# jzebedee/deltaq

Hardware: AMD Instinct MI355X
Metric: MB of text suffix-sorted per second (bit-exact SA) (higher is better)
Workload: dtype u8 text / u64 keys / int32 SA; 1 GPU; 256 MiB uniform-random bytes per GPU (splitmix64 seed 0x5EED0003+rank), int32 SA; bytes_per_gpu=268435456, residency=text and SA resident in HBM, rounds_after_initial_sort=1

## Files before the change

### deltaq_amd/csrc/dq_flags.h

```cpp
#pragma once

#include <algorithm>
#include <cstdint>
#include <cstdlib>
#include <cstring>
#include <optional>
#include <string>

namespace dq {

struct Flags {
    bool debug = false;
    std::optional<int> trace;
    std::optional<int> hip_device;
    std::optional<int> numa_bind;
    std::optional<std::string> fault;
    std::optional<int> small_n;
    std::optional<int> no_many;
    std::optional<int> mid_many_min;
    std::optional<int> no_large_many;
    std::optional<int> large_many_min;
    std::optional<int> no_diff_many;
    std::optional<int> no_diff_mid_many;
    std::optional<int> diff_mid_many_min;
    std::optional<int> no_diff_large;
    std::optional<int> diff_large_min;
    std::optional<int> diff_large_table;
    std::optional<int> no_index_many;
    std::optional<int> index_many_min;
    std::optional<int> index_many_threads;
    std::optional<int> no_index_large;
    std::optional<int> index_large_min;
    std::optional<int> no_check_many;
    std::optional<int> no_bwt_many;
    std::optional<int> no_mtf_many;
    std::optional<int> no_huff_many;
    std::optional<int> mtf_short_max;
    std::optional<int> unbz2_one_start;
    bool no_list_buffers = false;
    bool text_copy = false;
    bool assume_doubled = false;
    bool no_twins = false;
    bool no_period_hint = false;
    std::optional<int> xcd_group;
    std::optional<int> packed;
    std::optional<int> key_bytes;
    std::optional<int> coded;
    std::optional<int> split;
    bool no_bucket = false;
    std::optional<int> bucket;
    std::optional<int> bucket_keybits;
    std::optional<int> bucket_ext;
    std::optional<int> bucket_tile;
    std::optional<int> bucket_slots;
    std::optional<int> tie_settle;
    bool old_first_pass = false;
    bool no_fused_ties = false;
    std::optional<int> sparse;
    std::optional<int> binned_isa;
    bool no_binned_isa = false;
    std::optional<int> runs;
    bool no_small = false;
    bool no_wide_small = false;
    bool no_first_small = false;
    std::optional<int> mid_groups;
    bool no_l_shift = false;
    bool no_upd_words = false;
    std::optional<int> upd_bin;
    std::optional<int> upd_bin_min;
    std::optional<int> upd_window;
    std::optional<int> chain_steps;
    bool no_chain = false;
    bool force_rshift = false;
    std::optional<int> tail_max;
    std::optional<int> pair_chains;
    std::optional<int> pair_chains_min;
    std::optional<int> pair_maxg;
    std::optional<int> late_runs_min;
    bool no_late_runs = false;
    std::optional<int> run_period;
    bool search_wave = false;
    std::optional<int> search_ptab;
    bool no_wave_windows = false;
    bool no_poll = false;
    bool no_second_stage = false;
    std::optional<int> win_min;
    std::optional<int> win_second;
// ... 45 lines not shown
    f.no_diff_mid_many = num("DQ_NO_DIFF_MID_MANY", 0, 1);
    f.diff_mid_many_min = num("DQ_DIFF_MID_MANY_MIN", 1);
    f.no_diff_large = num("DQ_NO_DIFF_LARGE", 0, 1);
    f.diff_large_min = num("DQ_DIFF_LARGE_MIN", 1);
    f.diff_large_table = num("DQ_DIFF_LARGE_TABLE", 0, 1);
    f.no_index_many = num("DQ_NO_INDEX_MANY", 0, 1);
    f.index_many_min = num("DQ_INDEX_MANY_MIN", 1);
    f.index_many_threads = num("DQ_INDEX_MANY_THREADS");
    f.no_index_large = num("DQ_NO_INDEX_LARGE", 0, 1);
    f.index_large_min = num("DQ_INDEX_LARGE_MIN", 1);
    f.no_check_many = num("DQ_NO_CHECK_MANY", 0, 1);
    f.no_bwt_many = num("DQ_NO_BWT_MANY", 0, 1);
    f.no_mtf_many = num("DQ_NO_MTF_MANY", 0, 1);
    f.no_huff_many = num("DQ_NO_HUFF_MANY", 0, 1);
    f.mtf_short_max = num("DQ_MTF_SHORT_MAX", 0);
    f.unbz2_one_start = num("DQ_UNBZ2_ONE_START", 0, 1);
    f.no_list_buffers = on("DQ_NO_LIST_BUFFERS");
    f.text_copy = on("DQ_TEXT_COPY");
    f.assume_doubled = on("DQ_ASSUME_DOUBLED");
    f.no_twins = on("DQ_NO_TWINS");
    f.no_period_hint = on("DQ_NO_PERIOD_HINT");

    f.xcd_group = num("DQ_XCD_GROUP", 0, 64);
    f.packed = num("DQ_PACKED");
    f.key_bytes = num("DQ_KEY_BYTES", 1, 8);
    f.coded = num("DQ_CODED");
    f.split = num("DQ_SPLIT");
    f.no_bucket = on("DQ_NO_BUCKET");
    f.bucket = num("DQ_BUCKET");
    f.bucket_keybits = num("DQ_BUCKET_KEYBITS");
    f.bucket_ext = num("DQ_BUCKET_EXT");
    f.bucket_tile = num("DQ_BUCKET_TILE", 0, 1);
    f.bucket_slots = num("DQ_BUCKET_SLOTS", 0, 1);
    f.tie_settle = num("DQ_TIE_SETTLE", 0, 1);
    f.old_first_pass = on("DQ_OLD_FIRST_PASS");
    f.no_fused_ties = on("DQ_NO_FUSED_TIES");
    f.sparse = num("DQ_SPARSE");
    f.binned_isa = num("DQ_BINNED_ISA");
    f.no_binned_isa = on("DQ_NO_BINNED_ISA");
    f.runs = num("DQ_RUNS");

    f.no_small = on("DQ_NO_SMALL");
    f.no_wide_small = on("DQ_NO_WIDE_SMALL");
    f.no_first_small = on("DQ_NO_FIRST_SMALL");
    f.mid_groups = num("DQ_MID_GROUPS");
    f.no_l_shift = on("DQ_NO_L_SHIFT");
    f.no_upd_words = on("DQ_NO_UPD_WORDS");
    f.upd_bin = num("DQ_UPD_BIN", 0, 2);
    f.upd_bin_min = num("DQ_UPD_BIN_MIN", 1);
    f.upd_window = num("DQ_UPD_WINDOW");
    f.chain_steps = num("DQ_CHAIN_STEPS");
    f.no_chain = on("DQ_NO_CHAIN");
    f.force_rshift = on("DQ_FORCE_RSHIFT");

    f.tail_max = num("DQ_TAIL_MAX", 0);
    f.pair_chains = num("DQ_PAIR_CHAINS");
    f.pair_chains_min = num("DQ_PAIR_CHAINS_MIN", 1);
    f.pair_maxg = num("DQ_PAIR_MAXG", 2);
    f.late_runs_min = num("DQ_LATE_RUNS_MIN", 1);
    f.no_late_runs = on("DQ_NO_LATE_RUNS");
    f.run_period = num("DQ_RUN_PERIOD", 1);

    f.search_wave = on("DQ_SEARCH_WAVE");
    f.search_ptab = num("DQ_SEARCH_PTAB");
    f.no_wave_windows = on("DQ_NO_WAVE_WINDOWS");
    f.no_poll = on("DQ_NO_POLL");
// ... 79 lines not shown
```

### deltaq_amd/csrc/dq_round0.h

```cpp
#pragma once
#include "dq_sort_passes.h"
#include "dq_alpha_code.h"
#include "dq_ties.h"
#include "dq_bucket_sort.h"
#include "dq_xcd_rank.h"
#include "dq_slot_rank.h"

namespace dq {
namespace {

constexpr int64_t kSgShortList = 1 << 20;
inline int mid_group_cap(int64_t list_len)
{
    if (const std::optional<int> g = flags().mid_groups) {
        return *g >= 1024 ? 1024 : *g >= 512 ? 512 : *g >= 256 ? 256 : 0;
    }
    return list_len >= kSgShortList ? 512 : 1024;
}
inline bool small_round_usable(int64_t n, int64_t mm, bool third_list_buffer)
{
    const Flags &F = flags();
    return !F.no_small && n < (1ll << 32) && (mm * 2 <= n || (third_list_buffer && !F.no_wide_small));
}

// ... 45 lines not shown
    int digit_tables(int kb, bool coded_keys)
    {
        if (coded_keys) {
            const int hblocks = (int)std::min<int64_t>(kHistBlocks, ((n >> 2) + kHistThreads - 1) / kHistThreads + 1);
            DQ_TRY(L.begin(DQ_K_RADIX_HIST, n, n));
            HIP_TRY(hipMemsetAsync(w.hist_partial, 0, (size_t)kMaxPasses * kRadixSize * 8, st));
            hipLaunchKernelGGL(text_coded_hist_kernel, dim3(hblocks), dim3(kHistThreads), 0, st,
                               reinterpret_cast<const uint32_t *>(w.text), n, (const uint16_t *)w.codetab,
                               reinterpret_cast<unsigned long long *>(w.hist_partial));
            hipLaunchKernelGGL(radix_hist_scan_kernel, dim3(kMaxPasses), dim3(kHistScanThreads), 0, st,
                               (const unsigned long long *)w.hist_partial, w.digit_offset);
            HIP_TRY(hipGetLastError());
            return L.end();
        }
        hipLaunchKernelGGL(text_digit_offsets_kernel, dim3(kb), dim3(kBlock), 0, st,
                           (const int64_t *)w.bytehist, (const uint8_t *)w.text, n, kb, w.digit_offset);
        HIP_TRY(hipGetLastError());
        return DQ_OK;
    }

    int prepare()
    {
        int blocks = (int)std::min<int64_t>(1024, ((n >> 4) + kBlock - 1) / kBlock + 1);
        unsigned long long *xcd_hist = n >= kRound0MinN ? reinterpret_cast<unsigned long long *>(w.bytehist + kXcdHistAt) : nullptr;
        if (xcd_hist) blocks = (blocks + kXcds - 1) / kXcds * kXcds;
        HIP_TRY(hipMemsetAsync(w.bytehist, 0, (size_t)(kXcdHistAt + (xcd_hist ? kXcds * kRadixSize : 0)) * 8, L.st));
        LAUNCH(L, DQ_K_TEXT_HIST, n, n,
               hipLaunchKernelGGL(text_hist_kernel, dim3(blocks + 1), dim3(kBlock), 0, L.st,
                                  text_src ? text_src : (const uint8_t *)w.text, n, reinterpret_cast<unsigned long long *>(w.bytehist),
                                  reinterpret_cast<unsigned long long *>(w.bytehist + 256), text_src ? w.text : (uint8_t *)nullptr,
                                  xcd_hist));
        HIP_TRY(hipMemcpyAsync(c.pinned, w.bytehist, (256 + 10) * 8, hipMemcpyDeviceToHost, L.st));
        HIP_TRY(hipEventRecord(c.readback, L.st));
        constexpr int kEarlyPasses = 3;
        DQ_TRY(prepare_status<IdxT>(L, w, n, kEarlyPasses));
        if (n >= kRound0MinN) HIP_TRY(hipMemsetAsync(w.Vb, 0, (size_t)(tie_words() + 1) * 8, L.st));
        HIP_TRY(hipEventSynchronize(c.readback));
        const Flags &F = flags();
        s = TextStats(c.pinned, n);
        ib = s.ib;
        k = choose_key_bytes(s, F);
        DQ_TRY(prepare_status<IdxT>(L, w, n, k.kb, kEarlyPasses));
        bool hist_deferred = false;
        if (coded_keys_tried(s, F, k)) {
            AlphaCode code;
            if (build_alpha_code(s.hist, &code) && (code.avg_len <= kCodedMaxAvgLen || F.coded)) {
                uint16_t *stage = reinterpret_cast<uint16_t *>(c.pinned + 512);
                memcpy(stage, code.tab, sizeof(code.tab));
                HIP_TRY(hipMemcpyAsync(w.codetab, stage, sizeof(code.tab), hipMemcpyHostToDevice, L.st));
                coded = true;
                hist_deferred = split_round0_wanted(n, k, (int)wb, F);
                if (F.trace) fprintf(stderr, "[dq] coded round 0: %d symbols, %.2f bits per byte\n", code.sigma, code.avg_len);
            }
        }
        if (hist_deferred) return DQ_OK;
        if (!coded && plan_bucketed(s, F, k, coded, (int)wb).applies) return DQ_OK;
        return digit_tables(k.kb, coded);
    }

    int passes(int &cur, uint32_t *ebits = nullptr, uint64_t *seam_tab = nullptr)
    {
        const int kb = k.kb;
        if (k.packed) {
            DQ_TRY(rank_pass<IdxT, kTextPacked>(L, w, text64(), (const IdxT *)nullptr, K[1], (IdxT *)nullptr, n, 0, kb, ib));
            cur = 1;
            for (int p = 1; p < kb; ++p) {
                if (p == kb - 1 && ebits)
                    DQ_TRY(rank_pass<IdxT, kKeysLastTies>(L, w, K[cur], (const IdxT *)nullptr, (uint64_t *)nullptr, d_sa, n, p,
                                                          kb, ib, ebits, seam_tab));
                else if (p == kb - 1)
                    DQ_TRY(rank_pass<IdxT, kKeysLast>(L, w, K[cur], (const IdxT *)nullptr, K[cur ^ 1], d_sa, n, p, kb, ib));
                else
                    DQ_TRY(rank_pass<IdxT, kKeys>(L, w, K[cur], (const IdxT *)nullptr, K[cur ^ 1], (IdxT *)nullptr, n, p, kb, ib));
                cur ^= 1;
            }
            return DQ_OK;
        }
        DQ_TRY(with_bool(coded, [&](auto kCoded) -> int {
            return rank_pass<IdxT, kText, decltype(kCoded)::value>(L, w, text64(), (const IdxT *)nullptr, K[1], V[1], n, 0, kb);
        }));
        cur = 1;
        for (int p = 1; p < kb; ++p) {
            DQ_TRY(rank_pass<IdxT, kPairs>(L, w, K[cur], V[cur], K[cur ^ 1], V[cur ^ 1], n, p, kb));
            cur ^= 1;
        }
        return DQ_OK;
    }

    int collect_ties(uint32_t *ebits, const uint64_t *seam_tab, uint64_t *act_rank, bool *overflow, uint64_t *fin_rank,
                     bool seams = true, int64_t h_fin = -1, bool settle = false)
// ... 102 lines not shown
                                  keys, w.Va, cnt));
        o.keys_ready = with_key2;
        o.list_ungrouped = true;
        return DQ_OK;
    }

    int bucketed(bool *done)
    {
        *done = false;
        const Flags &F = flags();
        const BucketPlan b = plan_bucketed(s, F, k, coded, (int)wb);
        if (!b.applies) return DQ_OK;
        const int kb = k.kb, keybits = b.keybits, lowbits = b.lowbits;
        const SlotPlan sp = bucket_slots_fit(s, b, (int)wb);
        const FinishTiles ft = plan_finish_tiles(b, n, F, sp.fits);
        static_assert(sizeof(SlotRankCtl) <= (size_t)kHistBlocks * kMaxPasses * kRadixSize * 4, "the cursors live in the histogram scratch");
        const bool slots = bucket_slots_wanted(sp, ft, F) && (uint64_t)sp.words <= slot_span_words_of(w) &&
                           (size_t)(2 * kSlotBuckets + 5) * 4 <= finish_bounds_entries(n) * 8;
        uint32_t *slot_base = reinterpret_cast<uint32_t *>(w.bkt_bounds), *slot_out = slot_base + kSlotBuckets + 4;
        SlotRankCtl *sctl = reinterpret_cast<SlotRankCtl *>(w.hist_partial);
        const int first = slots ? 0 : 1;
        uint8_t *E[2] = {reinterpret_cast<uint8_t *>(w.Va), reinterpret_cast<uint8_t *>(w.Va) + align_up((size_t)n)};
        uint32_t *ebits = reinterpret_cast<uint32_t *>(w.Vb);
        TieCounters *ctr = reinterpret_cast<TieCounters *>(w.totals + 6);
        BucketFlags *bflags = reinterpret_cast<BucketFlags *>(&ctr->overflow);
        hipLaunchKernelGGL(text_digit_offsets_kernel, dim3(b.bbytes), dim3(kBlock), 0, st,
                           (const int64_t *)w.bytehist, (const uint8_t *)w.text, n, b.bbytes, w.digit_offset,
                           b.xcd_pass ? (const int64_t *)(w.bytehist + kXcdHistAt) : nullptr, b.xcd_pass ? w.xcd_offset : nullptr);
        HIP_TRY(hipGetLastError());
        if (slots) {
            if (F.trace)
                fprintf(stderr, "[dq] second pass into bucket slots: %d x %d slots of %lld words (n=%lld)\n", sp.first, sp.second,
                        (long long)b.X, (long long)n);
            HIP_TRY(hipMemsetAsync(sctl, 0, sizeof(SlotRankCtl), st));
            hipLaunchKernelGGL(slot_plan_kernel, dim3(kRadixSize + 1), dim3(kBlock), 0, st, (const int64_t *)w.bytehist, b.X, slot_base);
            HIP_TRY(hipGetLastError());
        }
        if (c.ncu <= 0) {
            int v = 0;
            c.ncu = hipDeviceGetAttribute(&v, hipDeviceAttributeMultiprocessorCount, c.dev) == hipSuccess && v > 0 ? v : 256;
        }
        if (b.xcd_pass) {
            if (F.trace) fprintf(stderr, "[dq] XCD-local first pass (n=%lld, eighths of %lld)\n", (long long)n, (long long)xcd_eighth(n));
            if (sizeof(XcdRankCtl) > w.ctl_status_stride) return fail(DQ_ERR_HIP, "status buffer too small");
            LAUNCH(L, DQ_K_RADIX_RANK, n, n * (1 + 8),
                   hipLaunchKernelGGL(xcd_text_rank_kernel, dim3((unsigned)std::min<int64_t>(c.ncu, (n + kXcdTileN - 1) / kXcdTileN)),
                                      dim3(kXcdRankThreads), 0, st, reinterpret_cast<const uint32_t *>(w.text), K[first], n,
                                      ib + lowbits, keybits, ib, (const int64_t *)w.xcd_offset,
                                      reinterpret_cast<XcdRankCtl *>(w.ctl_status)));
        } else {
            DQ_TRY(b.ext ? rank_pass_ext<IdxT, kTextPackedExt>(L, w, text64(), (const uint8_t *)nullptr, K[1], E[1], n, 0, ib, ib + lowbits, keybits)
                       : rank_pass<IdxT, kTextPacked>(L, w, text64(), (const IdxT *)nullptr, K[first], (IdxT *)nullptr, n, 0, kb, ib,
                                                      nullptr, nullptr, ib + lowbits, keybits));
        }
        if (slots) {
            const int groups = resident_groups(&c.slot_rank_groups, (const void *)slot_rank_kernel, kSlotRankThreads, c.dev);
            LAUNCH(L, DQ_K_RADIX_RANK, n, n * 16,
                   hipLaunchKernelGGL(slot_rank_kernel, dim3((unsigned)std::min<int64_t>(groups, (n + kSlotTileN - 1) / kSlotTileN)),
                                      dim3(kSlotRankThreads), 0, st, (const uint64_t *)K[0], K[1], n, ib + lowbits + 8, ib + lowbits,
                                      (const int64_t *)w.digit_offset, (const uint32_t *)slot_base, sctl, bflags));
        }
        for (int p = 1; p < b.bbytes && !slots; ++p) {
            DQ_TRY(b.ext ? rank_pass_ext<IdxT, kKeysExt>(L, w, K[p & 1], E[p & 1], K[(p & 1) ^ 1], E[(p & 1) ^ 1], n, p, ib, ib + lowbits + 8 * p, keybits)
                       : rank_pass<IdxT, kKeys>(L, w, K[p & 1], (const IdxT *)nullptr, K[(p & 1) ^ 1], (IdxT *)nullptr, n, p, kb, ib,
                                                nullptr, nullptr, ib + lowbits + 8 * p, keybits));
        }
        uint64_t *Ks = slots ? K[1] : K[b.bbytes & 1], *Kfree = slots ? K[0] : K[(b.bbytes & 1) ^ 1];
        const uint8_t *Es = b.ext ? E[b.bbytes & 1] : nullptr;
        if (F.trace)
            fprintf(stderr, "[dq] bucket finish: %s geometry, %lld tiles of up to %lld words cut every %lld %s (n=%lld)\n", ft.fine ? "fine" : "coarse",
                    (long long)ft.ntiles, (long long)ft.cap, (long long)(ft.by_id ? ft.g : ft.Cf), ft.by_id ? "buckets" : "words", (long long)n);
        if ((size_t)ft.ntiles + 1 > finish_bounds_entries(n)) return fail(DQ_ERR_HIP, "tile bounds buffer too small");
        if (slots) {
            LAUNCH(L, DQ_K_BUCKET_SORT, ft.ntiles, ft.ntiles * 16,
                   hipLaunchKernelGGL(slot_out_kernel, dim3(kRadixSize), dim3(kSlotOutThreads), 0, st, sctl->cursor, (uint32_t)b.X,
                                      (const int64_t *)(w.digit_offset + kRadixSize) , n, slot_out, bflags));
            auto kernel = bucket_sort_kernel<IdxT, false, BktFine, true>;
            const int groups = resident_groups(&c.bkt_slot_groups[sizeof(IdxT) == 8], (const void *)kernel, BktFine::threads, c.dev);
            LAUNCH(L, DQ_K_BUCKET_SORT, n, n * (8 + wb) + n / 8,
                   hipLaunchKernelGGL(kernel, dim3((unsigned)std::min<int64_t>(ft.ntiles, groups)), dim3(BktFine::threads), 0, st,
                                      (const uint64_t *)Ks, ib, lowbits, (const int64_t *)nullptr, ft.ntiles, d_sa, ebits, bflags,
                                      (const uint8_t *)nullptr, (const uint32_t *)slot_base, (const uint32_t *)sctl->cursor, (const uint32_t *)slot_out));
        } else if (ft.by_id) {
            const int64_t nbuckets = (int64_t)1 << (8 * b.bbytes);
            LAUNCH(L, DQ_K_BUCKET_SORT, ft.ntiles, ft.ntiles * 16 * 8,
                   hipLaunchKernelGGL(bucket_bounds_by_id_kernel, dim3((unsigned)((nbuckets + 1 + kBlock - 1) / kBlock)), dim3(kBlock), 0,
                                      st, (const uint64_t *)Ks, n, ib + lowbits, ft.g, b.X, nbuckets, ft.ntiles, w.bkt_bounds, bflags));
        } else {
            LAUNCH(L, DQ_K_BUCKET_SORT, ft.ntiles, ft.ntiles * 16 * 8,
                   hipLaunchKernelGGL(bucket_bounds_kernel, dim3((unsigned)((ft.ntiles + 1 + kBlock - 1) / kBlock)), dim3(kBlock), 0,
                                      st, (const uint64_t *)Ks, n, ib + lowbits, ft.Cf, b.X, ft.ntiles, w.bkt_bounds, bflags));
        }
        auto finish = [&](auto kExt, auto geometry) -> int {
// ... 151 lines not shown
            }
            *done = true;
            return DQ_OK;
        }
    }

    int run()
    {
        const Flags &F = flags();
        int cur = 0;
        DQ_TRY(prepare());
        const int kb = k.kb;
        o.runs = plan_runs(s, F, (int)wb, period_hint);
        V[kb & 1] = d_sa;
        V[(kb & 1) ^ 1] = w.Va;
        o.Vr[0] = w.Va; o.Vr[1] = w.Vb;
        o.rbits = ib;
        o.h = kb;
        bool done = false;
        DQ_TRY(bucketed(&done));
        if (done) return DQ_OK;
        if (fused_ties_wanted(n, k, F)) {
            uint32_t *ebits = reinterpret_cast<uint32_t *>(w.Vb);
            uint64_t *seam_tab = reinterpret_cast<uint64_t *>(reinterpret_cast<char *>(w.Vb) +
                                                              align_up((size_t)(tie_words() + 1) * 8));
            DQ_TRY(passes(cur, ebits, seam_tab));
            bool overflow = false;
            DQ_TRY(collect_ties(ebits, seam_tab, K[cur], &overflow, K[cur ^ 1]));
            o.fin_done = !overflow && o.m <= o.fin_cap;
            if (!overflow) {
                o.Kr[0] = K[cur]; o.Kr[1] = K[cur ^ 1];
                return DQ_OK;
            }
            HIP_TRY(hipMemsetAsync(w.ctl_status + (size_t)(kb - 1) * w.ctl_status_stride, 0, w.ctl_status_stride, st));
            DQ_TRY(rank_pass<IdxT, kKeysLast>(L, w, K[cur ^ 1], (const IdxT *)nullptr, K[cur], d_sa, n, kb - 1, kb, ib));
        } else {
            bool split_done = false;
            const bool split_wanted = split_round0_wanted(n, k, (int)wb, F);
            if (split_wanted && (!o.runs.runs_wanted || F.split)) {
                DQ_TRY(split(&split_done));
            }
            if (split_wanted && !split_done) {
                DQ_TRY(digit_tables(kb, coded));
                DQ_TRY(prepare_status<IdxT>(L, w, n, kb));
            }
            if (split_done) {
                cur = 1;
            } else {
                DQ_TRY(passes(cur));
            }
        }
        const int kshift0 = k.packed ? ib : 0;
        const DenseGuess guess = dense_guess(n, k);
        int64_t tied_pairs = 0;
        if (guess == DenseGuess::kTakeSample) {
            HIP_TRY(hipMemsetAsync(w.totals + 2, 0, 8, st));
            hipLaunchKernelGGL(sample_ties_kernel, dim3(kTieSamples / kBlock), dim3(kBlock), 0, st,
                               (const uint64_t *)K[cur], n, kshift0, kTieSamples, w.totals + 2);
            HIP_TRY(hipGetLastError());
            HIP_TRY(hipMemcpyAsync(c.pinned, w.totals + 2, 8, hipMemcpyDeviceToHost, st));
            HIP_TRY(hipStreamSynchronize(st));
            tied_pairs = c.pinned[0];
        }
        o.dense_built = predict_dense(guess, tied_pairs, F);
        if (o.dense_built && binned_isa_pays(n, F)) {
            o.Kr[0] = K[cur]; o.Kr[1] = K[cur ^ 1];
            return build_isa_binned(K[cur], K[cur ^ 1], kshift0);
// ... 10 lines not shown
```

### deltaq_amd/csrc/dq_round0_plan.h

```cpp
#pragma once
#include <algorithm>
#include <cmath>
#include <cstddef>
#include <cstdint>

#include "dq_flags.h"

namespace dq {

constexpr int kKgramSamples = 1024;
constexpr int kBktCap = 12288;
constexpr int kBktCapFine = 6144;
constexpr int kSplitTop = 512;
constexpr int kSplitSub = 512;
constexpr int kSplitBuckets = kSplitTop * kSplitSub;
constexpr int kFinCap = 2048;
constexpr int64_t kSplitMinN = 5ll << 20;
constexpr int64_t kCodedMinN = 8ll << 20;
constexpr double kCodedMaxAvgLen = 5.8;
constexpr int kTieSamples = 4096;
constexpr int64_t kRound0MinN = 1 << 16;

inline int index_bits(int64_t n) { return n <= 1 ? 1 : 64 - __builtin_clzll((uint64_t)(n - 1)); }

// ... 160 lines not shown
};

inline SlotPlan bucket_slots_fit(const TextStats &s, const BucketPlan &b, int idx_bytes)
{
    SlotPlan p;
    if (!b.applies || b.bbytes != 2 || b.ext) return p;
    p.first = s.sigma;
    p.second = s.sigma + (s.hist[0] == 0 ? 1 : 0);
    p.words = (int64_t)p.first * p.second * b.X;
    p.fits = p.words <= slot_span_words(s.n, idx_bytes) && p.words < ((int64_t)1 << 32);
    return p;
}

inline void slot_bases(const int64_t *hist , int64_t X, uint32_t *base )
{
    int ra[257], rb[257];
    ra[0] = rb[0] = 0;
    for (int d = 0; d < 256; ++d) {
        ra[d + 1] = ra[d] + (hist[d] > 0 ? 1 : 0);
        rb[d + 1] = rb[d] + (hist[d] > 0 || d == 0 ? 1 : 0);
    }
    for (int A = 0; A < 256; ++A)
        for (int B = 0; B < 256; ++B)
            base[A * 256 + B] = (uint32_t)(X * ((int64_t)ra[A] * rb[256] + (hist[A] > 0 ? rb[B] : 0)));
    base[65536] = (uint32_t)(X * ra[256] * rb[256]);
}

inline bool bucket_slots_wanted(const SlotPlan &p, const FinishTiles &t, const Flags &F)
{
    if (F.bucket_slots && *F.bucket_slots == 0) return false;
    return p.fits && t.fine && t.by_id && t.g == 1;
}

inline size_t finish_bounds_entries(int64_t n)
{
    const size_t by_words = (size_t)n / (kBktCapFine / 2) + 4;
    return n < kRound0MinN ? by_words : std::max<size_t>(by_words, 65536 + 4);
}

inline bool fused_ties_wanted(int64_t n, KeyPlan k, const Flags &F)
{
    return k.packed && k.kb >= 2 && n >= kRound0MinN && !F.no_fused_ties && !F.sparse;
}

enum class DenseGuess { kNeither, kGuessDense, kTakeSample };

inline DenseGuess dense_guess(int64_t n, KeyPlan k)
{
    if (n < kRound0MinN || k.packed || k.kb != 8) return DenseGuess::kNeither;
    return n < (8 << 20) ? DenseGuess::kGuessDense : DenseGuess::kTakeSample;
}

inline bool predict_dense(DenseGuess g, int64_t tied_pairs, const Flags &F)
{
    if (F.sparse) return *F.sparse == 0;
    return g == DenseGuess::kGuessDense || (g == DenseGuess::kTakeSample && tied_pairs * 12 > kTieSamples);
}

inline bool binned_isa_pays(int64_t n, const Flags &F)
{
    const bool pays = F.binned_isa ? *F.binned_isa != 0 : n > (32ll << 20);
    return pays && n >= kRound0MinN && 2 * index_bits(n) <= 63 && !F.no_binned_isa;
}

struct RunPlan {
    bool runs_wanted = false;
// ... 18 lines not shown
```

### deltaq_amd/csrc/dq_slot_rank.h

```cpp
#pragma once
#include "dq_bucket_sort.h"
#include "dq_xcd_rank.h"

namespace dq {

constexpr int kSlotBuckets = 1 << 16;

struct SlotRankCtl {
    uint32_t ticket[kXcds];
    uint32_t pad[64 - kXcds];
    uint32_t cursor[kSlotBuckets];
};

static __global__ __launch_bounds__(kBlock) void slot_plan_kernel(const int64_t *__restrict__ bytehist, int64_t X,
                                                           uint32_t *__restrict__ slot_base )
{
    __shared__ int tmp[kWavesPerBlock];
    __shared__ int s_rank, s_present;
    const int d = threadIdx.x, A = blockIdx.x;
    const int pa = bytehist[d] > 0 ? 1 : 0, pb = (pa || d == 0) ? 1 : 0;
    int na, nb;
    const int ra = block_excl_sum(pa, tmp, &na);
    __syncthreads();
    const int rb = block_excl_sum(pb, tmp, &nb);
    if (A == kRadixSize) {
        if (d == 0) slot_base[kSlotBuckets] = (uint32_t)(X * na * nb);
        return;
    }
    if (d == A) { s_rank = ra; s_present = pa; }
    __syncthreads();
    slot_base[A * kRadixSize + d] = (uint32_t)(X * ((int64_t)s_rank * nb + (s_present ? rb : 0)));
}

constexpr int kSlotOutThreads = kRadixSize;
static __global__ __launch_bounds__(kSlotOutThreads) void slot_out_kernel(uint32_t *__restrict__ count , uint32_t X,
                                                                   const int64_t *__restrict__ first_offset , int64_t n,
                                                                   uint32_t *__restrict__ out ,
                                                                   BucketFlags *__restrict__ flags)
{
    static_assert(kSlotOutThreads == kBlock, "block_excl_sum scans kBlock values");
    __shared__ uint32_t tmp[kWavesPerBlock];
    const int A = blockIdx.x, B = threadIdx.x;
    int64_t lo = first_offset[A], hi = A + 1 < kRadixSize ? first_offset[A + 1] : n;
    lo = lo < 0 ? 0 : (lo > n ? n : lo);
    hi = hi < lo ? lo : (hi > n ? n : hi);
    const uint32_t room = (uint32_t)(hi - lo);
    const uint32_t raw = count[A * kRadixSize + B];
    const uint32_t c = min(raw, X);
    uint32_t total;
    const uint32_t excl = block_excl_sum(c, tmp, &total);
    const uint32_t place = min(excl, room);
    const uint32_t kept = min(c, room - place);
    if (kept != raw) {
        atomicOr(&flags->overflow, 2ull);
        count[A * kRadixSize + B] = kept;
    }
    out[A * kRadixSize + B] = (uint32_t)lo + place;
    if (A == kRadixSize - 1 && B == kRadixSize - 1) out[kSlotBuckets] = (uint32_t)n;
}

#ifdef DQ_SLOT_PHASE_TIMING
__device__ long long *g_slot_ts = nullptr;
__device__ unsigned int g_slot_ts_next = 0;
#define DQ_SLOT_PHASE(i) do { if (threadIdx.x == 0 && g_slot_ts) g_slot_ts[(long long)ts_row * 8 + (i)] = clock64(); } while (0)
#else
#define DQ_SLOT_PHASE(i) do { } while (0)
#endif

constexpr int kSlotRankThreads = 1024;
constexpr int kSlotRankItems = 12;
constexpr int kSlotTileN = kSlotRankThreads * kSlotRankItems;

static __global__ __launch_bounds__(kSlotRankThreads, 1) void slot_rank_kernel(
    const uint64_t *__restrict__ kin , uint64_t *__restrict__ wout, int64_t n,
    int shift , int bshift ,
    const int64_t *__restrict__ region , const uint32_t *__restrict__ slot_base ,
    SlotRankCtl *__restrict__ ctl, BucketFlags *__restrict__ flags)
{
    constexpr int kThreads = kSlotRankThreads, kItems = kSlotRankItems, kTileN = kSlotTileN;
    constexpr int kPerXcd = kRadixSize / kXcds;
    __shared__ __attribute__((aligned(16))) uint64_t exch[kTileN];
    __shared__ uint32_t cnt[kRadixSize];
    __shared__ uint32_t tile_base[kRadixSize];
    __shared__ uint32_t gofs[kRadixSize];
    __shared__ uint32_t glim[kRadixSize];
    __shared__ uint32_t wtmp[kRadixSize / kWave];
    __shared__ uint32_t r_lo[kRadixSize], r_hi[kRadixSize], r_tiles[kRadixSize];
    __shared__ uint32_t xs[kXcds][kPerXcd + 1];
    __shared__ uint32_t s_lo, s_cnt;

    const int tid = threadIdx.x;
    const int w = tid >> 6;
    const int lane = lane_id();
    const uint32_t xcd = hw_xcc_id();

    if (tid < kRadixSize) {
        const int64_t lo = region[tid], hi = tid + 1 < kRadixSize ? region[tid + 1] : n;
        r_lo[tid] = (uint32_t)lo;
        r_hi[tid] = (uint32_t)hi;
        r_tiles[tid] = (uint32_t)((hi - lo + kTileN - 1) / kTileN);
        cnt[tid] = 0;
    }
    __syncthreads();
    if (tid < kXcds) {
        uint32_t run = 0;
        for (int j = 0; j < kPerXcd; ++j) { xs[tid][j] = run; run += r_tiles[tid + kXcds * j]; }
        xs[tid][kPerXcd] = run;
    }
    __syncthreads();

    int tried = 0;
    int32_t pend_e = -1;
// ... 121 lines not shown
```

### deltaq_amd/csrc/dq_sort_passes.h

```cpp
#pragma once
#include "dq_runtime.h"
#include "dq_round0_plan.h"
#include "dq_onesweep.h"
#include "dq_radix.h"
#include "dq_sa_kernels.h"
#include "dq_seg_fused.h"
#include "dq_small_groups.h"
#include "dq_runs.h"
#include "dq_isa_pairs.h"
#include "dq_split_round0.h"

namespace dq {
namespace {

constexpr int kSgChain = 8;

inline unsigned grid_for(int64_t items)
{
    return (unsigned)std::min<int64_t>((items + kBlock - 1) / kBlock, 256 * 16);
}

constexpr int64_t kSmallTileMaxM = 1ll << 20;
inline bool small_tiles(int64_t m) { return m <= kSmallTileMaxM; }
inline size_t status_tiles(size_t m)
{
    const size_t small = (m < (size_t)kSmallTileMaxM ? m : (size_t)kSmallTileMaxM) / 2048;
    return std::max(m / 8192, small) + 2;
}

template <typename IdxT>
struct Workspace {
    uint8_t *text;
    uint64_t *K0, *K1;
    IdxT *Va, *Vb, *ISA, *SAbuf;
    uint64_t *X;
    IdxT *Xs;
    int64_t *bkt_bounds;
    int64_t *totals;
    SmallGroupCounters *sg_ctr;
    uint32_t *hist_partial;
    uint16_t *codetab;
    uint32_t *pc_tiles;
    uint32_t *RL;
    uint32_t *run_lead, *run_carry;
    uint8_t *run_link;
    int64_t *digit_offset;
    int64_t *bytehist;
    int64_t *xcd_offset;
    char *ctl_status;
    size_t ctl_status_bytes;
    size_t ctl_status_stride;
    char *seg_status;
    size_t seg_status_bytes;
    uint64_t *sp_top, *sp_sub;
    unsigned long long *sp_cnt_a, *sp_cursor_a, *sp_cursor_b;
    int64_t *sp_off, *sp_out_base, *sp_ovf_src, *sp_ovf_dst;
    uint64_t *sp_low;
    uint8_t *sp_pure;
    uint32_t *sp_tile_first;
    ScanPart *sp_part;
    SplitCtl *sp_ctl;
    size_t slot_span_words;
    size_t bytes;
};

template <typename IdxT>
inline uint64_t slot_span_words_of(const Workspace<IdxT> &w) { return (uint64_t)w.slot_span_words; }

template <typename IdxT>
Workspace<IdxT> carve(char *base, int64_t n, bool with_sa, bool lists)
{
    Workspace<IdxT> w{};
    size_t off = 0;
    auto take = [&](size_t b) { char *p = base ? base + off : nullptr; off += align_up(b); return p; };
    const size_t un = (size_t)n;
    w.text = (uint8_t *)take(un + 64);
    w.K0 = (uint64_t *)take((un + 2) * 8);
    const size_t k1_at = off;
    w.K1 = (uint64_t *)take((un + 2) * 8);
    const bool adjacent = off == k1_at + align_up((un + 2) * 8);
    w.Va = (IdxT *)take((un + 2) * sizeof(IdxT));
    w.slot_span_words = adjacent ? (off - k1_at) / 8 : 0;
    w.Vb = (IdxT *)take((un + 2) * sizeof(IdxT));
    w.ISA = (IdxT *)take(un * sizeof(IdxT));
// ... 31 lines not shown
        w.sp_off = (int64_t *)take((size_t)(kSplitTop + 1) * 8);
        w.sp_out_base = (int64_t *)take((size_t)(kSplitBuckets + 1) * 8);
        w.sp_ovf_src = (int64_t *)take((size_t)kSplitBuckets * 8);
        w.sp_ovf_dst = (int64_t *)take((size_t)kSplitBuckets * 8);
        w.sp_low = (uint64_t *)take((size_t)kSplitBuckets * 8);
        w.sp_pure = (uint8_t *)take((size_t)kSplitBuckets);
        w.sp_tile_first = (uint32_t *)take((size_t)(kSplitTop + 1) * 4);
        w.sp_part = (ScanPart *)take((size_t)kScanBlocks * sizeof(ScanPart));
        w.sp_ctl = (SplitCtl *)take(sizeof(SplitCtl));
    }
    w.bytes = off;
    return w;
}

constexpr uint64_t kWsReserve = 1ull << 30;

template <typename IdxT>
bool with_list_buffers(int64_t n, bool with_sa, uint64_t avail)
{
    return n < (1ll << 32) && carve<IdxT>(nullptr, n, with_sa, true).bytes <= avail;
}

template <typename IdxT, int kMode, bool kSmall = false> struct RankCfg {
    static constexpr bool kExtra = (kMode == kTextPackedExt || kMode == kKeysExt);
    static constexpr bool kWords = (kMode == kTextPacked || kMode == kKeys || kMode == kKeysLast || kMode == kKeysLastTies || kExtra);
    static constexpr int kThreads = kSmall ? 256 : 512;
    static constexpr int kItems = kSmall ? 8 : kExtra ? 20 : kWords ? 24 : (sizeof(IdxT) == 4 ? 20 : 16);
    static constexpr int kMinWaves = 2;
    static constexpr int kRounds = 2;
    static constexpr bool kLdsMatch = kWords;
    static constexpr bool kAtomicBase = (kMode == kTextPacked || kMode == kText || kMode == kTextPackedExt);
};

template <typename IdxT>
int prepare_status(Launcher &L, Workspace<IdxT> &w, int64_t m, int passes, int from = 0)
{
    const size_t word = m < (1ll << 30) ? 4 : 8;
    const size_t stride = align_up(256 + status_tiles((size_t)m) * kRadixSize * word);
    if ((size_t)passes * stride > w.ctl_status_bytes) return fail(DQ_ERR_HIP, "status buffer too small");
    w.ctl_status_stride = stride;
    if (passes > from) HIP_TRY(hipMemsetAsync(w.ctl_status + (size_t)from * stride, 0, (size_t)(passes - from) * stride, L.st));
    return DQ_OK;
}

inline uint32_t spin_bound() { return t_fault.spin ? 0u : kSpinLimit; }

inline int xcd_tile_group() { return flags().xcd_group.value_or(8); }

template <typename IdxT, typename StatusT, int kMode, bool kCoded = false, bool kSmall = false>
int launch_rank_pass(Launcher &L, Workspace<IdxT> &w, const uint64_t *kin, const IdxT *vin,
                     uint64_t *kout, IdxT *vout, int64_t m, int pass, int kb, int ib,
                     uint32_t *ebits = nullptr, uint64_t *seam_tab = nullptr, int shift_override = -1,
                     int keybits = 0)
{
    using Cfg = RankCfg<IdxT, kMode, kSmall>;
    constexpr int kItems = Cfg::kItems;
    constexpr int kThreads = Cfg::kThreads;
    constexpr int kTileN = kThreads * kItems;
    const int64_t ntiles = (m + kTileN - 1) / kTileN;
    const int64_t wb = (int64_t)sizeof(IdxT);
    char *area = w.ctl_status + (size_t)pass * w.ctl_status_stride;
    OnesweepCtl *ctl = reinterpret_cast<OnesweepCtl *>(area);
    StatusT *status = reinterpret_cast<StatusT *>(area + 256);
    if (256 + (size_t)ntiles * kRadixSize * sizeof(StatusT) > w.ctl_status_stride)
        return fail(DQ_ERR_HIP, "status buffer too small");
    const int64_t alg = kMode == kPairs ? 2 * (8 + wb) : kMode == kText ? 1 + 8 + wb
                      : kMode == kTextPacked ? 1 + 8 : kMode == kKeys ? 16 : kMode == kKeysLastTies ? 8 + wb : 16 + wb;
    const int64_t alg_extra = kMode == kKeysLastTies ? m / 8 + ntiles * kRadixSize * 16 : 0;
    LAUNCH(L, DQ_K_RADIX_RANK, m, m * alg + alg_extra,
           hipLaunchKernelGGL((radix_rank_kernel<IdxT, StatusT, kItems, kMode, Cfg::kMinWaves, kThreads,
                                                 false, Cfg::kLdsMatch, Cfg::kRounds, Cfg::kAtomicBase, kCoded>),
                              dim3((unsigned)ntiles), dim3(kThreads), 0, L.st, kin, vin, kout, vout, m,
                              shift_override >= 0 ? shift_override : pass * kRadixBits + ib,
                              keybits > 0 ? keybits : 8 * kb, ib,
                              (const int64_t *)(w.digit_offset + pass * kRadixSize), status, ctl, w.totals + 1,
                              ebits, seam_tab, (const uint16_t *)w.codetab, xcd_tile_group(), spin_bound()));
    return DQ_OK;
}

template <typename Fn>
int with_status_word(int64_t m, Fn fn)
{
    return m < (1ll << 30) ? fn(uint32_t{}) : fn(uint64_t{});
}

template <typename IdxT, int kMode>
int rank_pass_ext(Launcher &L, Workspace<IdxT> &w, const uint64_t *kin, const uint8_t *ein, uint64_t *kout, uint8_t *eout,
                  int64_t m, int pass, int ib, int shift, int keybits)
{
    static_assert(kMode == kTextPackedExt || kMode == kKeysExt, "extra-byte modes");
    using Cfg = RankCfg<IdxT, kMode>;
    constexpr int kTileN = Cfg::kThreads * Cfg::kItems;
    const int64_t ntiles = (m + kTileN - 1) / kTileN;
    char *area = w.ctl_status + (size_t)pass * w.ctl_status_stride;
    OnesweepCtl *ctl = reinterpret_cast<OnesweepCtl *>(area);
    return with_status_word(m, [&](auto status_tag) -> int {
        using StatusT = decltype(status_tag);
        StatusT *status = reinterpret_cast<StatusT *>(area + 256);
        if (256 + (size_t)ntiles * kRadixSize * sizeof(StatusT) > w.ctl_status_stride)
            return fail(DQ_ERR_HIP, "status buffer too small");
        LAUNCH(L, DQ_K_RADIX_RANK, m, m * (kMode == kTextPackedExt ? 1 + 8 + 1 : 18),
               hipLaunchKernelGGL((radix_rank_kernel<IdxT, StatusT, Cfg::kItems, kMode, Cfg::kMinWaves, Cfg::kThreads, false,
                                                     Cfg::kLdsMatch, Cfg::kRounds, Cfg::kAtomicBase, false, uint8_t>),
                                  dim3((unsigned)ntiles), dim3(Cfg::kThreads), 0, L.st, kin, ein, kout, eout, m, shift, keybits, ib,
                                  (const int64_t *)(w.digit_offset + pass * kRadixSize), status, ctl, w.totals + 1,
                                  (uint32_t *)nullptr, (uint64_t *)nullptr, (const uint16_t *)w.codetab, xcd_tile_group(), spin_bound()));
        return DQ_OK;
    });
}

template <typename IdxT, int kMode, bool kCoded = false>
int rank_pass(Launcher &L, Workspace<IdxT> &w, const uint64_t *kin, const IdxT *vin, uint64_t *kout,
              IdxT *vout, int64_t m, int pass, int kb, int ib = 0, uint32_t *ebits = nullptr,
              uint64_t *seam_tab = nullptr, int shift_override = -1, int keybits = 0)
{
    if (small_tiles(m))
        return launch_rank_pass<IdxT, uint32_t, kMode, kCoded, true>(L, w, kin, vin, kout, vout, m, pass, kb, ib, ebits,
                                                                     seam_tab, shift_override, keybits);
    return with_status_word(m, [&](auto word) -> int {
        return launch_rank_pass<IdxT, decltype(word), kMode, kCoded>(L, w, kin, vin, kout, vout, m, pass, kb, ib, ebits, seam_tab,
                                                                     shift_override, keybits);
    });
}

template <int kPasses>
void launch_hist(hipStream_t st, int blocks, const uint64_t *keys, int64_t m, uint32_t *acc_area, int shift0 = 0)
{
// ... 88 lines not shown
```

Measured before the change: 93560 MB/s.

## Track zeroed status areas and skip redundant memsets on the predicted route

Adds a host-side record of which per-pass status/control areas are already zeroed, so each radix pass claims and zeroes its area only when needed instead of blanket memsets. Before the histogram readback it guesses (from a uniform histogram model) whether the bucket-slots route will run, and if so zeroes only the XCD control header rather than three full pass areas. The slot control cursor/ticket reset moves into slot_plan_kernel, removing a separate memset. The slot rank kernel is also templated on geometry without changing the default. Risk: bookkeeping errors could leave a status area dirty and corrupt the onesweep lookback.

```diff
diff --git a/deltaq_amd/csrc/dq_flags.h b/deltaq_amd/csrc/dq_flags.h
--- a/deltaq_amd/csrc/dq_flags.h
+++ b/deltaq_amd/csrc/dq_flags.h
@@ -53,6 +53,7 @@
     std::optional<int> bucket_ext;
     std::optional<int> bucket_tile;
     std::optional<int> bucket_slots;
+    std::optional<int> early_zero;
     std::optional<int> tie_settle;
     bool old_first_pass = false;
     bool no_fused_ties = false;
@@ -164,6 +165,7 @@
     f.bucket_ext = num("DQ_BUCKET_EXT");
     f.bucket_tile = num("DQ_BUCKET_TILE", 0, 1);
     f.bucket_slots = num("DQ_BUCKET_SLOTS", 0, 1);
+    f.early_zero = num("DQ_EARLY_ZERO", 0, 1);
     f.tie_settle = num("DQ_TIE_SETTLE", 0, 1);
     f.old_first_pass = on("DQ_OLD_FIRST_PASS");
     f.no_fused_ties = on("DQ_NO_FUSED_TIES");
diff --git a/deltaq_amd/csrc/dq_round0.h b/deltaq_amd/csrc/dq_round0.h
--- a/deltaq_amd/csrc/dq_round0.h
+++ b/deltaq_amd/csrc/dq_round0.h
@@ -101,15 +101,23 @@
                                   xcd_hist));
         HIP_TRY(hipMemcpyAsync(c.pinned, w.bytehist, (256 + 10) * 8, hipMemcpyDeviceToHost, L.st));
         HIP_TRY(hipEventRecord(c.readback, L.st));
+        const Flags &F = flags();
         constexpr int kEarlyPasses = 3;
-        DQ_TRY(prepare_status<IdxT>(L, w, n, kEarlyPasses));
         if (n >= kRound0MinN) HIP_TRY(hipMemsetAsync(w.Vb, 0, (size_t)(tie_words() + 1) * 8, L.st));
+        w.status.reset();
+        DQ_TRY(prepare_status<IdxT>(L, w, n, 0));
+        const bool guess_slots = slots_route_guess(n, (int)wb, F);
+        const int early = F.early_zero ? (*F.early_zero != 0 ? 2 : 0) : guess_slots ? 1 : 2;
+        if (F.trace && n >= kRound0MinN)
+            fprintf(stderr, "[dq] early zero: %s (guess: %s; n=%lld)\n", early == 2 ? "three passes" : early == 1 ? "first-pass cursors only" : "nothing",
+                    guess_slots ? "slots" : "another route", (long long)n);
+        if (early == 2) DQ_TRY(prepare_status<IdxT>(L, w, n, kEarlyPasses));
+        if (early == 1) DQ_TRY(claim_xcd_ctl());
         HIP_TRY(hipEventSynchronize(c.readback));
-        const Flags &F = flags();
         s = TextStats(c.pinned, n);
         ib = s.ib;
         k = choose_key_bytes(s, F);
-        DQ_TRY(prepare_status<IdxT>(L, w, n, k.kb, kEarlyPasses));
+        if (early == 2) DQ_TRY(prepare_status<IdxT>(L, w, n, k.kb));
         bool hist_deferred = false;
         if (coded_keys_tried(s, F, k)) {
             AlphaCode code;
@@ -124,7 +132,15 @@
         }
         if (hist_deferred) return DQ_OK;
         if (!coded && plan_bucketed(s, F, k, coded, (int)wb).applies) return DQ_OK;
+        DQ_TRY(prepare_status<IdxT>(L, w, n, k.kb));
         return digit_tables(k.kb, coded);
+    }
+
+    int claim_xcd_ctl()
+    {
+        if (sizeof(XcdRankCtl) > w.ctl_status_stride) return fail(DQ_ERR_HIP, "status buffer too small");
+        if (w.status.claim_head()) HIP_TRY(hipMemsetAsync(w.ctl_status, 0, sizeof(XcdRankCtl), L.st));
+        return DQ_OK;
     }
 
     int passes(int &cur, uint32_t *ebits = nullptr, uint64_t *seam_tab = nullptr)
@@ -293,9 +309,10 @@
             if (F.trace)
                 fprintf(stderr, "[dq] second pass into bucket slots: %d x %d slots of %lld words (n=%lld)\n", sp.first, sp.second,
                         (long long)b.X, (long long)n);
-            HIP_TRY(hipMemsetAsync(sctl, 0, sizeof(SlotRankCtl), st));
-            hipLaunchKernelGGL(slot_plan_kernel, dim3(kRadixSize + 1), dim3(kBlock), 0, st, (const int64_t *)w.bytehist, b.X, slot_base);
+            hipLaunchKernelGGL(slot_plan_kernel, dim3(kRadixSize + 1), dim3(kBlock), 0, st, (const int64_t *)w.bytehist, b.X, slot_base, sctl);
             HIP_TRY(hipGetLastError());
+        } else {
+            DQ_TRY(prepare_status<IdxT>(L, w, n, b.bbytes));
         }
         if (c.ncu <= 0) {
             int v = 0;
@@ -303,7 +320,8 @@
         }
         if (b.xcd_pass) {
             if (F.trace) fprintf(stderr, "[dq] XCD-local first pass (n=%lld, eighths of %lld)\n", (long long)n, (long long)xcd_eighth(n));
-            if (sizeof(XcdRankCtl) > w.ctl_status_stride) return fail(DQ_ERR_HIP, "status buffer too small");
+            DQ_TRY(claim_xcd_ctl());
+            w.status.wrote(0);
             LAUNCH(L, DQ_K_RADIX_RANK, n, n * (1 + 8),
                    hipLaunchKernelGGL(xcd_text_rank_kernel, dim3((unsigned)std::min<int64_t>(c.ncu, (n + kXcdTileN - 1) / kXcdTileN)),
                                       dim3(kXcdRankThreads), 0, st, reinterpret_cast<const uint32_t *>(w.text), K[first], n,
@@ -315,11 +333,13 @@
                                                       nullptr, nullptr, ib + lowbits, keybits));
         }
         if (slots) {
-            const int groups = resident_groups(&c.slot_rank_groups, (const void *)slot_rank_kernel, kSlotRankThreads, c.dev);
+            using G = RankCoarse;
+            auto kernel = slot_rank_kernel<G>;
+            const int groups = resident_groups(&c.slot_rank_groups, (const void *)kernel, G::threads, c.dev);
             LAUNCH(L, DQ_K_RADIX_RANK, n, n * 16,
-                   hipLaunchKernelGGL(slot_rank_kernel, dim3((unsigned)std::min<int64_t>(groups, (n + kSlotTileN - 1) / kSlotTileN)),
-                                      dim3(kSlotRankThreads), 0, st, (const uint64_t *)K[0], K[1], n, ib + lowbits + 8, ib + lowbits,
-                                      (const int64_t *)w.digit_offset, (const uint32_t *)slot_base, sctl, bflags));
+                   hipLaunchKernelGGL(kernel, dim3((unsigned)std::min<int64_t>(groups, (n + G::tile - 1) / G::tile)), dim3(G::threads), 0, st,
+                                      (const uint64_t *)K[0], K[1], n, ib + lowbits + 8, ib + lowbits, (const int64_t *)w.digit_offset,
+                                      (const uint32_t *)slot_base, sctl, bflags));
         }
         for (int p = 1; p < b.bbytes && !slots; ++p) {
             DQ_TRY(b.ext ? rank_pass_ext<IdxT, kKeysExt>(L, w, K[p & 1], E[p & 1], K[(p & 1) ^ 1], E[(p & 1) ^ 1], n, p, ib, ib + lowbits + 8 * p, keybits)
@@ -537,7 +557,6 @@
                 o.Kr[0] = K[cur]; o.Kr[1] = K[cur ^ 1];
                 return DQ_OK;
             }
-            HIP_TRY(hipMemsetAsync(w.ctl_status + (size_t)(kb - 1) * w.ctl_status_stride, 0, w.ctl_status_stride, st));
             DQ_TRY(rank_pass<IdxT, kKeysLast>(L, w, K[cur ^ 1], (const IdxT *)nullptr, K[cur], d_sa, n, kb - 1, kb, ib));
         } else {
             bool split_done = false;
diff --git a/deltaq_amd/csrc/dq_round0_plan.h b/deltaq_amd/csrc/dq_round0_plan.h
--- a/deltaq_amd/csrc/dq_round0_plan.h
+++ b/deltaq_amd/csrc/dq_round0_plan.h
@@ -216,6 +216,61 @@
     return p.fits && t.fine && t.by_id && t.g == 1;
 }
 
+inline bool slots_route_guess(int64_t n, int idx_bytes, const Flags &F)
+{
+    if (n < kRound0MinN || index_bits(n) > 31) return false;
+    TextStats s;
+    s.n = n;
+    s.ib = index_bits(n);
+    for (int b = 0; b < 256; ++b) s.hist[b] = n / 256 + (b < n % 256 ? 1 : 0);
+    s.sigma = 256;
+    s.cmax = s.hist[0];
+    s.h0 = 8.0;
+    const KeyPlan k = choose_key_bytes(s, F);
+    const BucketPlan b = plan_bucketed(s, F, k, coded_keys_tried(s, F, k), idx_bytes);
+    if (!b.applies || !b.xcd_pass) return false;
+    if (F.bucket && F.bucket_tile && *F.bucket_tile == 1 && F.bucket_slots && *F.bucket_slots == 1) return b.bbytes == 2;
+    const SlotPlan sp = bucket_slots_fit(s, b, idx_bytes);
+    return bucket_slots_wanted(sp, plan_finish_tiles(b, n, F, sp.fits), F);
+}
+
+struct StatusRecord {
+    static constexpr int kPasses = 8;
+    size_t stride = 0;
+    uint32_t clean = 0;
+    bool head = false;
+
+    void reset() { stride = 0; clean = 0; head = false; }
+    void set_stride(size_t s) { if (s != stride) { stride = s; clean = 0; head = false; } }
+    template <typename Fn>
+    int claim(int from, int to, Fn zero)
+    {
+        to = std::min(to, kPasses);
+        for (int p = std::max(from, 0); p < to;) {
+            if (clean >> p & 1u) { ++p; continue; }
+            int q = p;
+            while (q < to && !(clean >> q & 1u)) ++q;
+            if (const int rc = zero(p, q - p)) return rc;
+            for (int i = p; i < q; ++i) clean |= 1u << i;
+            if (p == 0) head = true;
+            p = q;
+        }
+        return 0;
+    }
+    bool claim_head()
+    {
+        const bool need = !head && !(clean & 1u);
+        head = true;
+        return need;
+    }
+    void wrote(int p)
+    {
+        if (p < 0 || p >= kPasses) return;
+        clean &= ~(1u << p);
+        if (p == 0) head = false;
+    }
+};
+
 inline size_t finish_bounds_entries(int64_t n)
 {
     const size_t by_words = (size_t)n / (kBktCapFine / 2) + 4;
diff --git a/deltaq_amd/csrc/dq_slot_rank.h b/deltaq_amd/csrc/dq_slot_rank.h
--- a/deltaq_amd/csrc/dq_slot_rank.h
+++ b/deltaq_amd/csrc/dq_slot_rank.h
@@ -13,11 +13,15 @@
 };
 
 static __global__ __launch_bounds__(kBlock) void slot_plan_kernel(const int64_t *__restrict__ bytehist, int64_t X,
-                                                           uint32_t *__restrict__ slot_base )
+                                                           uint32_t *__restrict__ slot_base ,
+                                                           SlotRankCtl *__restrict__ ctl)
 {
+    static_assert(kBlock == kRadixSize && kXcds <= kBlock, "a thread per second byte and per ticket");
     __shared__ int tmp[kWavesPerBlock];
     __shared__ int s_rank, s_present;
     const int d = threadIdx.x, A = blockIdx.x;
+    if (A < kRadixSize) ctl->cursor[A * kRadixSize + d] = 0;
+    else if (d < kXcds) ctl->ticket[d] = 0;
     const int pa = bytehist[d] > 0 ? 1 : 0, pb = (pa || d == 0) ? 1 : 0;
     int na, nb;
     const int ra = block_excl_sum(pa, tmp, &na);
@@ -67,17 +71,24 @@
 #define DQ_SLOT_PHASE(i) do { } while (0)
 #endif
 
-constexpr int kSlotRankThreads = 1024;
-constexpr int kSlotRankItems = 12;
-constexpr int kSlotTileN = kSlotRankThreads * kSlotRankItems;
-
-static __global__ __launch_bounds__(kSlotRankThreads, 1) void slot_rank_kernel(
+template <int kThreads, int kItems, int kGroupsPerCu>
+struct RankGeometry {
+    static constexpr int threads = kThreads, items = kItems, groups = kGroupsPerCu;
+    static constexpr int tile = kThreads * kItems;
+    static constexpr int min_waves = kGroupsPerCu > 1 ? kGroupsPerCu * kThreads / (kWave * 4) : 1;
+    static_assert(kThreads % kWave == 0 && kThreads >= kRadixSize, "whole waves, a thread per digit");
+};
+using RankCoarse = RankGeometry<1024, 12, 1>;
+using RankFine = RankGeometry<512, 12, 2>;
+
+template <typename G = RankCoarse>
+static __global__ __launch_bounds__(G::threads, G::min_waves) void slot_rank_kernel(
     const uint64_t *__restrict__ kin , uint64_t *__restrict__ wout, int64_t n,
     int shift , int bshift ,
     const int64_t *__restrict__ region , const uint32_t *__restrict__ slot_base ,
     SlotRankCtl *__restrict__ ctl, BucketFlags *__restrict__ flags)
 {
-    constexpr int kThreads = kSlotRankThreads, kItems = kSlotRankItems, kTileN = kSlotTileN;
+    constexpr int kThreads = G::threads, kItems = G::items, kTileN = G::tile;
     constexpr int kPerXcd = kRadixSize / kXcds;
     __shared__ __attribute__((aligned(16))) uint64_t exch[kTileN];
     __shared__ uint32_t cnt[kRadixSize];
diff --git a/deltaq_amd/csrc/dq_sort_passes.h b/deltaq_amd/csrc/dq_sort_passes.h
--- a/deltaq_amd/csrc/dq_sort_passes.h
+++ b/deltaq_amd/csrc/dq_sort_passes.h
@@ -50,6 +50,7 @@
     char *ctl_status;
     size_t ctl_status_bytes;
     size_t ctl_status_stride;
+    StatusRecord status;
     char *seg_status;
     size_t seg_status_bytes;
     uint64_t *sp_top, *sp_sub;
@@ -147,14 +148,32 @@
     static constexpr bool kAtomicBase = (kMode == kTextPacked || kMode == kText || kMode == kTextPackedExt);
 };
 
-template <typename IdxT>
-int prepare_status(Launcher &L, Workspace<IdxT> &w, int64_t m, int passes, int from = 0)
+static_assert(StatusRecord::kPasses == kMaxPasses, "one bit per digit pass");
+template <typename IdxT>
+int prepare_status(Launcher &L, Workspace<IdxT> &w, int64_t m, int passes)
 {
     const size_t word = m < (1ll << 30) ? 4 : 8;
     const size_t stride = align_up(256 + status_tiles((size_t)m) * kRadixSize * word);
     if ((size_t)passes * stride > w.ctl_status_bytes) return fail(DQ_ERR_HIP, "status buffer too small");
     w.ctl_status_stride = stride;
-    if (passes > from) HIP_TRY(hipMemsetAsync(w.ctl_status + (size_t)from * stride, 0, (size_t)(passes - from) * stride, L.st));
+    w.status.set_stride(stride);
+    return w.status.claim(0, passes, [&](int first, int count) -> int {
+        HIP_TRY(hipMemsetAsync(w.ctl_status + (size_t)first * stride, 0, (size_t)count * stride, L.st));
+        return DQ_OK;
+    });
+}
+
+template <typename IdxT>
+int claim_status(Launcher &L, Workspace<IdxT> &w, int pass, char **area)
+{
+    if ((size_t)(pass + 1) * w.ctl_status_stride > w.ctl_status_bytes) return fail(DQ_ERR_HIP, "status buffer too small");
+    w.status.set_stride(w.ctl_status_stride);
+    DQ_TRY(w.status.claim(pass, pass + 1, [&](int first, int count) -> int {
+        HIP_TRY(hipMemsetAsync(w.ctl_status + (size_t)first * w.ctl_status_stride, 0, (size_t)count * w.ctl_status_stride, L.st));
+        return DQ_OK;
+    }));
+    w.status.wrote(pass);
+    *area = w.ctl_status + (size_t)pass * w.ctl_status_stride;
     return DQ_OK;
 }
 
@@ -174,7 +193,8 @@
     constexpr int kTileN = kThreads * kItems;
     const int64_t ntiles = (m + kTileN - 1) / kTileN;
     const int64_t wb = (int64_t)sizeof(IdxT);
-    char *area = w.ctl_status + (size_t)pass * w.ctl_status_stride;
+    char *area = nullptr;
+    DQ_TRY(claim_status<IdxT>(L, w, pass, &area));
     OnesweepCtl *ctl = reinterpret_cast<OnesweepCtl *>(area);
     StatusT *status = reinterpret_cast<StatusT *>(area + 256);
     if (256 + (size_t)ntiles * kRadixSize * sizeof(StatusT) > w.ctl_status_stride)
@@ -207,7 +227,8 @@
     using Cfg = RankCfg<IdxT, kMode>;
     constexpr int kTileN = Cfg::kThreads * Cfg::kItems;
     const int64_t ntiles = (m + kTileN - 1) / kTileN;
-    char *area = w.ctl_status + (size_t)pass * w.ctl_status_stride;
+    char *area = nullptr;
+    DQ_TRY(claim_status<IdxT>(L, w, pass, &area));
     OnesweepCtl *ctl = reinterpret_cast<OnesweepCtl *>(area);
     return with_status_word(m, [&](auto status_tag) -> int {
         using StatusT = decltype(status_tag);
```

After: 94200 MB/s (median of 6 runs). No clear change (+0.7%).
